# PixArt-alpha/PixArt-sigma

Hardware: AMD Instinct MI355X
Metric: denoising steps/sec (fwd+bwd) PixArt-Sigma-XL/2 1024px bs16 @1/2/4/8 GPU (higher is better)
Workload: dtype fp16; 1 GPU; PixArt-Sigma-XL/2 1024px training step (fwd+bwd+clip+AdamW), batch 16/GPU, L=300 text tokens, DP=1 RCCL all-reduce; model=PixArtMS_XL_2, global_batch=16, seq_len=4096, parallelism=dp1, grad_checkpoint=False, optimizer=adamw, text_lens=all 300

## Files before the change

### pixart_sigma_amd/csrc/gemm.hip

```cpp
#include <atomic>
#include "common.h"
#include "gemm_params.h"
#include "../../include/pixart_hip.h"
#include <cstdio>
#include <cstdlib>
#include <cstring>

namespace {
using namespace pxa;

constexpr int BM = 128, BN = 128, BK = 64;
constexpr int KC_BYTES = 128 * BK * 2;
constexpr int RC_STRIDE = (128 + 32) * 2;
constexpr int RC_BYTES = BK * RC_STRIDE;


template <bool KC>
__device__ __forceinline__ void g2r(const bf16_t* __restrict__ X, int ld, int r0, int R, int k0, int kend, uint4 (&reg)[4], int tid) {
#pragma unroll
  for (int i = 0; i < 4; i++) {
    const bf16_t* src;
    bool ok;
    if (KC) {
      int c = tid & 7, row = (tid >> 3) + 32 * i;
// ... 509 lines not shown
__device__ __forceinline__ void wait_vm_upto(int n) {
  if (n >= 6) wait_vmcnt<6>();
  else if (n == 4) wait_vmcnt<4>();
  else if (n == 2) wait_vmcnt<2>();
  else wait_vmcnt<0>();
}
#define PXA_SB() __builtin_amdgcn_sched_barrier(0)
#ifndef GEMM_ABL
#define GEMM_ABL 0
#endif
#if GEMM_ABL & 4
__device__ __forceinline__ void mfma_abl16(f32x4 (&q)[4], bf16x8 b0, bf16x8 a0, bf16x8 b1, bf16x8 a1) {
  q[0] = mfma16(b0, a0, q[0]); q[1] = mfma16(b1, a1, q[1]); q[2] = mfma16(b0, a1, q[2]); q[3] = mfma16(b1, a0, q[3]);
}
#endif
#ifndef GEMM_STORE_OVERLAP
#define GEMM_STORE_OVERLAP 1
#endif
#ifndef GEMM_M16
#define GEMM_M16 3
#endif
#ifndef GEMM_NT_STORE
#define GEMM_NT_STORE 0
#endif
#ifndef GEMM_M16_PRIO
#define GEMM_M16_PRIO 1
#endif
#ifndef GEMM_STAGGER
#define GEMM_STAGGER 0
#endif
#ifndef GEMM_EPI_EARLY
#define GEMM_EPI_EARLY 1
#endif
#ifndef GEMM_PHASE16
#define GEMM_PHASE16 -1
#endif

template <bool M16>
__device__ __forceinline__ int kc_swz(int row) { return M16 ? ((row >> 3) & 1) * 3 : (row >> 2) & 3; }
template <bool KC, bool M16 = false>
__device__ __forceinline__ const bf16_t* piece_ptr_rt(const bf16_t* __restrict__ X, int ld, int r0a, int r0b, int R, int q, int rows_log2) {
  if constexpr (KC) {
    const int row = q >> 2, c = (q & 3) ^ kc_swz<M16>(row);
    const int gr = (row < 256 ? r0a : r0b - 256) + row;
    return X + (size_t)min(gr, R - 1) * ld + c * 8;
  } else {
    const int sh = rows_log2 - 3, kr = q >> sh, cl = q & ((1 << sh) - 1);
    const int c = ((((cl >> 2) ^ (kr & 3)) << 2) | ((cl & 3) ^ (M16 ? ((kr >> 3) & 1) << 1 : 0)));
    const int col = c * 8;
    int gc = (col < 256 ? r0a : r0b - 256) + col;
    gc = gc < R ? gc : 0;
    return X + (size_t)kr * ld + gc;
  }
}
template <bool KC>
__device__ __forceinline__ bf16x8 frag_rt(const char* lds, int rbase, int ks, int lane, int rows_log2) {
  if constexpr (KC) {
    return frag_p<true, 256, 32>(lds, rbase, ks, lane);
  } else {
    const int gg = lane >> 4, tt = lane & 15, hi2 = gg >> 1;
    const int kr = ks * 16 + 8 * hi2 + (tt >> 2), col = rbase + 16 * (gg & 1) + (tt & 3) * 4;
    const int blk = col >> 5, inblk = (col & 31) * 2;
    const char* p0 = lds + (kr << (rows_log2 + 1)) + ((blk ^ (kr & 3)) << 6) + inblk;
    const char* p1 = lds + ((kr + 4) << (rows_log2 + 1)) + ((blk ^ ((kr + 4) & 3)) << 6) + inblk;
    return concat_tr(lds_tr_read(p0), lds_tr_read(p1));
  }
// ... 5 lines not shown
}
template <bool KC>
__device__ __forceinline__ bf16x8 frag16(const char* lds, int rbase, int lane, int rows_log2) {
  if constexpr (KC) {
    return frag16_kc(lds, rbase, lane);
  } else {
    const int gg = lane >> 4, tt = lane & 15;
    const int kr = 8 * gg + (tt >> 2), col = rbase + (tt & 3) * 4;
    const int blk = col >> 5, inblk = ((col & 31) * 2) ^ ((gg & 1) << 5);
    const char* p0 = lds + (kr << (rows_log2 + 1)) + ((blk ^ (kr & 3)) << 6) + inblk;
    const char* p1 = lds + ((kr + 4) << (rows_log2 + 1)) + ((blk ^ ((kr + 4) & 3)) << 6) + inblk;
    return concat_tr(lds_tr_read(p0), lds_tr_read(p1));
  }
}

#ifndef GEMM_TRACE
#define GEMM_TRACE 0
#endif
#if GEMM_TRACE
__device__ unsigned long long g_trace[12][8];
#define PXA_TR(k) do { if (blockIdx.x == 8 && tid == 0 && tr_i < 12) g_trace[tr_i][k] = __builtin_readcyclecounter(); } while (0)
#else
#define PXA_TR(k) do {} while (0)
#endif
__device__ unsigned g_sched[64][16];
__device__ unsigned g_sched_word[64][512];

template <int LAYOUT, int EPI, int RM, bool SEG = false>
__global__ __launch_bounds__(512) void gemm_pers_kernel(GemmParams p) {
  constexpr bool A_KC = (LAYOUT != 2), B_KC = (LAYOUT == 0);
  constexpr int NW = 8, TM = 4, TN = 2, BKT = 32, H1 = 2;
  constexpr bool PH16 = GEMM_PHASE16 < 0 ? (LAYOUT != 0) : (GEMM_PHASE16 != 0);
  constexpr bool M16 = ((GEMM_M16 >> LAYOUT) & 1) && !(GEMM_ABL & 4);
  constexpr int UNIT = 40960;
  extern __shared__ __attribute__((aligned(16))) char smem[];
  const int tid = threadIdx.x, lane = tid & 63, wave = __builtin_amdgcn_readfirstlane(tid >> 6), wm = wave >> 2, wn = wave & 3, hi = lane >> 5;
  const bool late = wave >= NW / 2;
  char* stg = smem + 3 * UNIT + wave * 4096;
  const int mt = (p.M + 255) / 256, ntf = p.N / 256, remn = p.N - ntf * 256;
  constexpr bool PAIR = (RM == 1), HALF = (RM == 2);
  const bool remcol = RM != 0 && remn > 0 && remn <= 128;
  const int ntp = remcol ? ntf : (p.N + 255) / 256;
  const int rem_pg = remcol ? (PAIR ? 4 : 8) : 0;
  const int per_group = 8 * ntp + rem_pg, tiles = mt * ntp + (remcol ? (PAIR ? (mt + 1) / 2 : mt) : 0), T = tiles * p.split;
  auto units_of = [&](int z) { return (min(p.K, (z + 1) * p.k_per_split) - z * p.k_per_split) / BKT; };

  int m0a = 0, m0b = 0, n0 = 0, z_ = 0;
  bool vt = false;
  const int xq = T / 8, xr = T % 8;
  auto xs = [&](int x) { return x * xq + min(x, xr); };
  auto xc = [&](int x) { return xq + (x < xr ? 1 : 0); };
  auto locate_g = [&](int Lg) {
    z_ = Lg / tiles;
    const int t = Lg - z_ * tiles;
    const int g = t / per_group, in_g = t - g * per_group, first_m = g * 8, gsz = min(mt - first_m, 8), nfull = gsz * ntp;
    if (in_g < nfull) { vt = false; m0a = (first_m + in_g % gsz) * 256; m0b = m0a; n0 = (in_g / gsz) * 256; }
    else if (PAIR) { vt = true; m0a = (first_m + 2 * (in_g - nfull)) * 256; m0b = m0a + 256; n0 = ntf * 256; }
    else if (HALF) { vt = true; m0a = (first_m + (in_g - nfull)) * 256; m0b = m0a; n0 = ntf * 256; }
  };
  const bool rev = LAYOUT != 2 && p.desc != 0;
  auto pos_of = [&](int x, int i) { return xs(x) + (rev ? xc(x) - 1 - i : i); };
  auto locate = [&](int L) { locate_g(pos_of(L % 8, L / 8)); };
  const bool DYN = p.sched_slot >= 0;
  const int myx = blockIdx.x % 8;
  unsigned* sched = g_sched[p.sched_slot & 63];
  unsigned* sched_lds = reinterpret_cast<unsigned*>(smem + 32768);
  unsigned* sched_glb = &g_sched_word[p.sched_slot & 63][blockIdx.x & 511];
  auto publish = [&](int v) {
    if (PAIR) { if (lane == 0) __hip_atomic_store(sched_glb, (unsigned)v, __ATOMIC_RELAXED, __HIP_MEMORY_SCOPE_AGENT); wait_vmcnt<0>(); }
    else { if (lane == 0) sched_lds[0] = (unsigned)v; asm volatile("s_waitcnt lgkmcnt(0)" ::: "memory"); }
  };
// ... 84 lines not shown
  auto issue_lo = [&]() __attribute__((always_inline)) {
#pragma unroll
    for (int i = 0; i < H1; i++) piece(i, s_lo);
    if (SEG) PXA_SEG_ADVANCE(seg_left0, tap_kx0, tap_ky0, tap_half0, pp[0], pp[1]);
    s_lo = (s_lo + 1) & 3;
  };
  auto issue_hi = [&]() __attribute__((always_inline)) {
    piece(2, s_hi);
    if (!(HALF && vt_pf)) piece(3, s_hi);
    if (PAIR && vt_pf) piece(4, s_hi);
    if (SEG && PAIR) { if (vt_pf) PXA_SEG_ADVANCE(seg_left1, tap_kx1, tap_ky1, tap_half1, pp[2], pp[3]); }
    s_hi = (s_hi + 1) & 3;
  };
#undef PXA_SEG_ADVANCE
  auto prefetch = [&]() __attribute__((always_inline)) {
    vt_pf = (RM != 0) && vt;
    const long k0 = (long)z_ * p.k_per_split;
    const bool vq = PAIR && vt, hq = HALF && vt;
    const int rla = vq ? 9 : 8, rlb = (vq || hq) ? 7 : 8;
    const int ln = opaque<LAYOUT == 1 || (EPI >= 2 && EPI != 7) || (GEMM_EPI_EARLY && RM == 2)>(lane);
#pragma unroll
    for (int i = 0; i < 5; i++) {
      const int id = wave + NW * i;
      const bool is_a = vq ? (i < 4) : (i < 2);
      const int pid = is_a ? id : (vq ? id - 32 : id - 16);
      if (vq || (hq ? i < 3 : i < 4)) {
        if (is_a) pp[i] = piece_ptr_rt<A_KC, M16>(p.A, p.lda, m0a, m0b, p.M, pid * 64 + ln, rla) + (A_KC ? k0 : k0 * p.lda);
        else pp[i] = piece_ptr_rt<B_KC, M16>(p.B, p.ldb, n0, n0, p.N, pid * 64 + ln, rlb) + (B_KC ? k0 : k0 * p.ldb);
      }
      st[i] = is_a ? stepA : stepB;
      dof[i] = (is_a ? 0 : (vq ? 32768 : 16384)) + pid * 1024;
    }
    s_lo = s_hi = 0;
    dma_count = 0;
    if (SEG) { seg_left0 = seg_left1 = p.k_seg; tap_kx0 = tap_kx1 = tap_ky0 = tap_ky1 = tap_half0 = tap_half1 = 0; }
    issue_lo(); issue_hi(); issue_lo(); issue_hi();
    if (nk_pf > 2) { issue_lo(); if (PH16) issue_hi(); }
  };
  prefetch();
  int tr_i = 0; (void)tr_i;
  int prev_stores = 0;

  while (true) {
    f32x16 acc[TM][TN];
    f32x4 acc4[2 * TM][2 * TN];
#pragma unroll
    for (int i = 0; i < TM; i++)
#pragma unroll
      for (int j = 0; j < TN; j++)
#pragma unroll
        for (int g = 0; g < 16; g++) acc[i][j][g] = 0.f;
#pragma unroll
    for (int i = 0; i < 2 * TM; i++)
#pragma unroll
      for (int j = 0; j < 2 * TN; j++) acc4[i][j] = f32x4{0.f, 0.f, 0.f, 0.f};
#if GEMM_ABL & 4
    f32x4 a4[TM][TN][4];
#pragma unroll
    for (int i = 0; i < TM; i++)
#pragma unroll
      for (int j = 0; j < TN; j++)
#pragma unroll
        for (int q = 0; q < 4; q++) a4[i][j][q] = f32x4{0.f, 0.f, 0.f, 0.f};
#endif
    const bool vtc = PAIR && vt, hfc = HALF && vt;
    const int a_rb = hfc ? (wave >> 1) * 64 : (vtc ? (wn >> 1) * 256 : 0) + wm * 128, b_rb = (vtc || hfc) ? (wn & 1) * 64 : wn * 64;
    const int rla = vtc ? 9 : 8, rlb = (vtc || hfc) ? 7 : 8, boff = vtc ? 32768 : 16384;
    const int mw = hfc ? m0a + a_rb : ((vtc && (wn >> 1)) ? m0b : m0a) + wm * 128, nw = n0 + b_rb;
    const int tm_eff = hfc ? 2 : TM;
    const int zw = z_;
    PXA_TR(0);
    if (GEMM_STORE_OVERLAP && LAYOUT != 2 && EPI != 3) {
      if (prev_stores == 40) wait_vmcnt<40>();
      else if (prev_stores == 36) wait_vmcnt<36>();
      else if (prev_stores == 32) wait_vmcnt<32>();
      else if (prev_stores == 28) wait_vmcnt<28>();
      else if (prev_stores == 24) wait_vmcnt<24>();
      else if (prev_stores == 20) wait_vmcnt<20>();
      else if (prev_stores == 16) wait_vmcnt<16>();
      else if (prev_stores == 12) wait_vmcnt<12>();
      else if (prev_stores == 8) wait_vmcnt<8>();
      else wait_vmcnt<0>();
    } else {
      wait_vmcnt<0>();
    }
    if (DYN && wave == 0) {
      publish(fetch_resolve());
    }
    __builtin_amdgcn_s_barrier();
    if (DYN) nxt = receive();
    if (late) __builtin_amdgcn_s_barrier();
    PXA_TR(1);
    constexpr bool EARLY = GEMM_EPI_EARLY && M16 && LAYOUT != 2;
    constexpr bool AUXA = EARLY && (EPI == 2 || EPI == 4 || EPI == 6) && !(GEMM_ABL & 16);
    typedef unsigned u32x2 __attribute__((ext_vector_type(2)));
    u32x2 axa[2][2][4];
    f32x4 bq[2 * TN];
    const bool has_bias = EARLY && p.bias != nullptr;
    auto bias_issue = [&]() {
      const int R4b = lane >> 4;
#pragma unroll
      for (int jn = 0; jn < 2 * TN; jn++) {
        const float* src = p.bias + min(nw + jn * 16 + 4 * R4b, p.N - 4);
        asm volatile("global_load_dwordx4 %0, %1, off" : "=v"(bq[jn]) : "v"(src) : "memory");
      }
    };
    auto aux_issue = [&](int i, u32x2 (&dst)[2][4]) {
      const int R4a = lane >> 4, c16a = lane & 15;
#pragma unroll
      for (int mh = 0; mh < 2; mh++)
#pragma unroll
        for (int jn = 0; jn < 4; jn++) {
          const int m = min(mw + i * 32 + 16 * mh + c16a, p.M - 1), n = min(nw + jn * 16 + 4 * R4a, p.N - 4);
          const bf16_t* src = p.aux + (size_t)m * p.ldaux + n;
          asm volatile("global_load_dwordx2 %0, %1, off" : "=v"(dst[mh][jn]) : "v"(src) : "memory");
        }
    };
    auto unit16 = [&](int t, auto rem_c, auto th_c) {
      constexpr int REM = decltype(rem_c)::value, TH = decltype(th_c)::value;
      const char* sA = smem + (t & 3) * UNIT;
      const char* sB = sA + boff;
      if constexpr (M16) {
        bf16x8 bq[2 * TN], aq[4 * TH];
#pragma unroll
        for (int j = 0; j < 2 * TN; j++) bq[j] = frag16<B_KC>(sB, b_rb + j * 16, lane, rlb);
#pragma unroll
        for (int i = 0; i < 4 * TH; i++) aq[i] = frag16<A_KC>(sA, a_rb + i * 16, lane, rla);
        if (REM >= 3) { issue_lo(); issue_hi(); }
        if (REM >= 3) { if (vtc) wait_vmcnt<10>(); else if (TH == 1) wait_vmcnt<6>(); else wait_vmcnt<8>(); }
        else if (REM == 2) { if (vtc) wait_vmcnt<5>(); else if (TH == 1) wait_vmcnt<3>(); else wait_vmcnt<4>(); }
        else if (REM == 1) wait_vmcnt<0>();
        asm volatile("s_waitcnt lgkmcnt(0)" ::: "memory");
        PXA_SB(); __builtin_amdgcn_s_barrier(); PXA_SB();
        if (GEMM_M16_PRIO && LAYOUT != 1) __builtin_amdgcn_s_setprio(1);
#pragma unroll
        for (int i = 0; i < 4 * TH; i++)
#pragma unroll
          for (int j = 0; j < 2 * TN; j++) acc4[i][j] = mfma16(bq[j], aq[i], acc4[i][j]);
        if (GEMM_M16_PRIO && LAYOUT != 1) __builtin_amdgcn_s_setprio(0);
        PXA_SB(); __builtin_amdgcn_s_barrier(); PXA_SB();
        return;
      }
      bf16x8 af[2][2 * TH], bf[2][TN];
#pragma unroll
      for (int ks = 0; ks < 2; ks++)
#pragma unroll
        for (int j = 0; j < TN; j++) bf[ks][j] = frag_rt<B_KC>(sB, b_rb + j * 32, ks, lane, rlb);
#pragma unroll
      for (int ks = 0; ks < 2; ks++)
#pragma unroll
        for (int i = 0; i < 2 * TH; i++) af[ks][i] = frag_rt<A_KC>(sA, a_rb + i * 32, ks, lane, rla);
      if (REM >= 3) { issue_lo(); issue_hi(); }
      if (REM >= 3) { if (vtc) wait_vmcnt<10>(); else if (TH == 1) wait_vmcnt<6>(); else wait_vmcnt<8>(); }
      else if (REM == 2) { if (vtc) wait_vmcnt<5>(); else if (TH == 1) wait_vmcnt<3>(); else wait_vmcnt<4>(); }
      else if (REM == 1) wait_vmcnt<0>();
      asm volatile("s_waitcnt lgkmcnt(0)" ::: "memory");
      PXA_SB(); __builtin_amdgcn_s_barrier(); PXA_SB();
      __builtin_amdgcn_s_setprio(1);
#if GEMM_ABL & 4
#pragma unroll
      for (int i = 0; i < 2 * TH; i++)
#pragma unroll
        for (int j = 0; j < TN; j++) mfma_abl16(a4[i][j], bf[0][j], af[0][i], bf[1][j], af[1][i]);
#else
#pragma unroll
      for (int ks = 0; ks < 2; ks++)
#pragma unroll
        for (int i = 0; i < 2 * TH; i++)
#pragma unroll
          for (int j = 0; j < TN; j++) acc[i][j] = mfma32(bf[ks][j], af[ks][i], acc[i][j]);
#endif
      __builtin_amdgcn_s_setprio(0);
      PXA_SB(); __builtin_amdgcn_s_barrier(); PXA_SB();
    };
    auto unit8 = [&](int t, auto rem_c, auto th_c) {
      constexpr int REM = decltype(rem_c)::value, TH = decltype(th_c)::value;
      const char* sA = smem + (t & 3) * UNIT;
      const char* sB = sA + boff;
      auto rest_a = [&]() { if (REM >= 2) issue_hi(); };
      auto rest_b = [&]() {
        if (REM >= 3) issue_lo();
        if (REM >= 3) { if (vtc) wait_vmcnt<7>(); else if (TH == 1) wait_vmcnt<5>(); else wait_vmcnt<6>(); }
        else if (REM == 2) { if (vtc) wait_vmcnt<5>(); else if (TH == 1) wait_vmcnt<3>(); else wait_vmcnt<4>(); }
        else if (REM == 1) wait_vmcnt<0>();
      };
      if constexpr (M16) {
        bf16x8 bq[2 * TN];
#pragma unroll
        for (int j = 0; j < 2 * TN; j++) bq[j] = frag16<B_KC>(sB, b_rb + j * 16, lane, rlb);
#pragma unroll
        for (int h = 0; h < 2; h++) {
          bf16x8 aq[2 * TH];
#pragma unroll
          for (int i = 0; i < 2 * TH; i++) aq[i] = frag16<A_KC>(sA, a_rb + (h * 2 * TH + i) * 16, lane, rla);
          if (h == 0) rest_a(); else rest_b();
          PXA_SB(); __builtin_amdgcn_s_barrier(); PXA_SB();
          if (GEMM_M16_PRIO) __builtin_amdgcn_s_setprio(1);
#pragma unroll
          for (int i = 0; i < 2 * TH; i++)
#pragma unroll
            for (int j = 0; j < 2 * TN; j++) acc4[h * 2 * TH + i][j] = mfma16(bq[j], aq[i], acc4[h * 2 * TH + i][j]);
          if (GEMM_M16_PRIO) __builtin_amdgcn_s_setprio(0);
          PXA_SB(); __builtin_amdgcn_s_barrier(); PXA_SB();
        }
        return;
      }
      bf16x8 af[2][TH], bf[2][TN];
#pragma unroll
      for (int ks = 0; ks < 2; ks++)
#pragma unroll
        for (int j = 0; j < TN; j++) bf[ks][j] = frag_rt<B_KC>(sB, b_rb + j * 32, ks, lane, rlb);
#pragma unroll
      for (int h = 0; h < 2; h++) {
#pragma unroll
        for (int ks = 0; ks < 2; ks++)
#pragma unroll
          for (int i = 0; i < TH; i++) af[ks][i] = frag_rt<A_KC>(sA, a_rb + (h * TH + i) * 32, ks, lane, rla);
        if (h == 0) rest_a(); else rest_b();
        PXA_SB(); __builtin_amdgcn_s_barrier(); PXA_SB();
        __builtin_amdgcn_s_setprio(1);
#if GEMM_ABL & 4
#pragma unroll
        for (int i = 0; i < TH; i++)
#pragma unroll
          for (int j = 0; j < TN; j++) mfma_abl16(a4[h * TH + i][j], bf[0][j], af[0][i], bf[1][j], af[1][i]);
#else
#pragma unroll
        for (int ks = 0; ks < 2; ks++)
#pragma unroll
// ... 10 lines not shown
    };
    auto run_units = [&](auto th_c) {
      int t = 0;
      for (; t < nk - 3; t++) unit(t, IntC<3>{}, th_c);
      if (nk >= 3) unit(t++, IntC<2>{}, th_c);
      unit(t++, IntC<1>{}, th_c);
      unit(t++, IntC<0>{}, th_c);
    };
    if (HALF && hfc) run_units(IntC<1>{}); else run_units(IntC<2>{});
#if GEMM_ABL & 4
#pragma unroll
    for (int i = 0; i < TM; i++)
#pragma unroll
      for (int j = 0; j < TN; j++)
#pragma unroll
        for (int g = 0; g < 16; g++) acc[i][j][g] = a4[i][j][g >> 2][g & 3];
#endif
    PXA_TR(2);
    if constexpr (LAYOUT != 2) {
      if (has_bias) bias_issue();
      if constexpr (AUXA) { aux_issue(0, axa[0]); aux_issue(1, axa[1]); }
    }
    if (!late) __builtin_amdgcn_s_barrier();
    PXA_TR(3);

    bool more = false;
    int pf_ops = 0;
    auto hand_over = [&]() {
      if (DYN) {
        more = nxt >= 0;
        if (more) {
          locate_g(nxt);
          nk_pf = units_of(z_);
          prefetch();
          fetch_issue();
        }
      } else {
        L += gridDim.x;
        more = L < T;
        if (more) {
          locate(L);
          nk_pf = units_of(z_);
          prefetch();
        }
      }
      if (more) pf_ops = dma_count;
    };
    const int le = opaque<LAYOUT == 1 || (EPI >= 2 && EPI != 7) || (GEMM_EPI_EARLY && RM == 2)>(lane);
    const int srow = le & 31;
    if constexpr (LAYOUT == 2) {
      hand_over();
      PXA_TR(4);
#pragma unroll
      for (int i = 0; i < TM; i++)
#pragma unroll
        for (int j = 0; j < TN; j++) {
          if constexpr (M16) {
#pragma unroll
            for (int mh = 0; mh < 2; mh++)
#pragma unroll
              for (int nh = 0; nh < 2; nh++) {
                const f32x4 a = acc4[2 * i + mh][2 * j + nh];
                const int row = 16 * mh + (lane & 15);
                *reinterpret_cast<float4*>(stg + row * 128 + (((4 * nh + (lane >> 4)) ^ (row & 7)) << 4)) = make_float4(a[0], a[1], a[2], a[3]);
              }
          } else {
#pragma unroll
          for (int q = 0; q < 4; q++)
            *reinterpret_cast<float4*>(stg + srow * 128 + (((q * 2 + hi) ^ (srow & 7)) << 4)) =
                make_float4(acc[i][j][q * 4], acc[i][j][q * 4 + 1], acc[i][j][q * 4 + 2], acc[i][j][q * 4 + 3]);
          }
          __builtin_amdgcn_s_waitcnt(0xc07f);
#pragma unroll
          for (int t4 = 0; t4 < 4; t4++) {
            const int row = t4 * 8 + (lane >> 3), ch = lane & 7;
// ... 54 lines not shown
      else if (allowed >= 24) wait_vmcnt<24>();
      else if (allowed >= 22) wait_vmcnt<22>();
      else if (allowed >= 20) wait_vmcnt<20>();
      else if (allowed >= 16) wait_vmcnt<16>();
      else if (allowed >= 12) wait_vmcnt<12>();
      else if (allowed >= 10) wait_vmcnt<10>();
      else if (allowed >= 9) wait_vmcnt<9>();
      else if (allowed >= 8) wait_vmcnt<8>();
      else if (allowed >= 4) wait_vmcnt<4>();
      else wait_vmcnt<0>();
    };
    auto aux_ready = [&](int allowed, u32x2 (&a)[2][4]) {
      wait_allow(allowed);
      asm volatile("" : "+v"(a[0][0]), "+v"(a[0][1]), "+v"(a[0][2]), "+v"(a[0][3]), "+v"(a[1][0]), "+v"(a[1][1]), "+v"(a[1][2]), "+v"(a[1][3]));
    };
    auto aux_apply = [&](int i, const u32x2 (&a)[2][4]) {
#pragma unroll
      for (int mh = 0; mh < 2; mh++)
#pragma unroll
        for (int jn = 0; jn < 4; jn++) {
          float a0, a1, a2f, a3;
          unpack_bf16x2(a[mh][jn][0], a0, a1); unpack_bf16x2(a[mh][jn][1], a2f, a3);
          f32x4& v = acc4[2 * i + mh][jn];
          if (act == 5) { v[0] += a0; v[1] += a1; v[2] += a2f; v[3] += a3; }
          else { v[0] *= a0; v[1] *= a1; v[2] *= a2f; v[3] *= a3; }
        }
    };
    hand_over();
    if constexpr (AUXA) {
      aux_ready(8 + pf_ops, axa[0]);
      if (has_bias) bias_apply();
      aux_apply(0, axa[0]);
      if (tm_eff > 2) aux_issue(2, axa[0]);
    } else {
      if (has_bias) { wait_allow(pf_ops); bias_apply(); }
    }
    PXA_TR(4);
    auto emit = [&](int j0, auto jw_c) {
      constexpr int JW = decltype(jw_c)::value, RB = JW * 64;
      constexpr int LPR = JW * 4, RPI = 64 / LPR, NST = 4 / (3 - JW);
      static_assert(!M16 || JW == 2, "16 x 16 accumulator tiles: the wave's 64 columns are one column group");
      const int R4 = le >> 4, c16 = le & 15;
      if (!EARLY) bias_add();
      float cs[8], sq[2] = {0.f, 0.f};
#pragma unroll
      for (int e = 0; e < 8; e++) cs[e] = 0.f;
      const int st_img = want_st ? mw / p.gn_img_rows : 0, st_base = st_img * p.gn_img_rows;
      const bool want_aux = !AUXA && (act == 2 || act == 4 || act == 5);
      const bool interior_a = mw + tm_eff * 32 <= p.M && nw + 64 <= p.N;
      uint2 ax[2][JW][4];
      auto load_aux = [&](int i, uint2 (&dst)[JW][4]) {
        if constexpr ((GEMM_ABL & 16) != 0) {
#pragma unroll
          for (int a_ = 0; a_ < JW; a_++)
#pragma unroll
            for (int b_ = 0; b_ < 4; b_++) dst[a_][b_] = make_uint2(OPERAND_ONE_X2, OPERAND_ONE_X2);
        } else if constexpr (M16) {
#pragma unroll
          for (int mh = 0; mh < 2; mh++)
#pragma unroll
            for (int jn = 0; jn < 4; jn++) {
              const int m = mw + i * 32 + 16 * mh + c16, n = nw + jn * 16 + 4 * R4;
              dst[mh][jn] = (m < p.M && n < p.N) ? *reinterpret_cast<const uint2*>(p.aux + (size_t)m * p.ldaux + n) : make_uint2(0u, 0u);
            }
        } else {
        const int m = mw + i * 32 + srow;
#pragma unroll
        for (int jj = 0; jj < JW; jj++)
#pragma unroll
          for (int q = 0; q < 4; q++) {
            const int n = nw + (j0 + jj) * 32 + 8 * q + 4 * hi;
            dst[jj][q] = (m < p.M && n < p.N) ? *reinterpret_cast<const uint2*>(p.aux + (size_t)m * p.ldaux + n) : make_uint2(0u, 0u);
          }
        }
      };
      auto finish4 = [&](int pass, float (&v)[4], auto&& put_back, const uint2& a2) {
        if (pass == 0 && act == 3) {
          float g[4];
#pragma unroll
          for (int e = 0; e < 4; e++) {
            if (GEMM_ABL & 64) { g[e] = v[e]; put_back(e, v[e]); }
            else put_back(e, gelu_tanh_both(v[e], g[e]));
            v[e] = g[e];
          }
        }
        if (pass == 1) {
          if (act == 1) {
#pragma unroll
            for (int e = 0; e < 4; e++) v[e] = gelu_tanh(v[e]);
          } else if (!AUXA && (act == 2 || act == 4 || act == 5)) {
            float a0, a1, a2f, a3;
            unpack_bf16x2(a2.x, a0, a1); unpack_bf16x2(a2.y, a2f, a3);
            if (act == 2) { a0 = gelu_tanh_grad(a0); a1 = gelu_tanh_grad(a1); a2f = gelu_tanh_grad(a2f); a3 = gelu_tanh_grad(a3); }
            if (act == 5) { v[0] += a0; v[1] += a1; v[2] += a2f; v[3] += a3; }
            else { v[0] *= a0; v[1] *= a1; v[2] *= a2f; v[3] *= a3; }
          }
        }
      };
      if (want_aux) load_aux(0, ax[0]);
#pragma unroll
      for (int i = 0; i < TM; i++) {
        if (i >= tm_eff) break;
        if (want_aux && i + 1 < tm_eff) load_aux(i + 1, ax[(i + 1) & 1]);
        if constexpr (AUXA) {
          if (i == 1) {
            aux_ready(interior_a ? (tm_eff > 2 ? 8 : 0) + pf_ops + 4 : 0, axa[1]);
            aux_apply(1, axa[1]);
            if (tm_eff > 3) aux_issue(3, axa[1]);
          } else if (i == 2) {
            aux_ready(interior_a ? 16 : 0, axa[0]);
            aux_apply(2, axa[0]);
          } else if (i == 3) {
            aux_ready(interior_a ? 8 : 0, axa[1]);
            aux_apply(3, axa[1]);
          }
        }
#pragma unroll
        for (int pass = 0; pass < 2; pass++) {
          if (pass == 0 && !dual) continue;
          if constexpr (M16) {
#pragma unroll
            for (int mh = 0; mh < 2; mh++)
#pragma unroll
              for (int jn = 0; jn < 4; jn++) {
                f32x4& a = acc4[2 * i + mh][jn];
                float v[4] = {a[0], a[1], a[2], a[3]};
                finish4(pass, v, [&](int e, float x) { a[e] = x; }, ax[i & 1][mh][jn]);
                const int row = 16 * mh + c16, ch = 2 * jn + (R4 >> 1);
                *reinterpret_cast<uint2*>(stg + row * RB + ((ch ^ (row & 7)) << 4) + (R4 & 1) * 8) = pack_bf16x4(v[0], v[1], v[2], v[3]);
              }
          } else {
#pragma unroll
          for (int jj = 0; jj < JW; jj++)
#pragma unroll
            for (int q = 0; q < 4; q++) {
              const int j = j0 + jj;
              float v[4] = {acc[i][j][q * 4], acc[i][j][q * 4 + 1], acc[i][j][q * 4 + 2], acc[i][j][q * 4 + 3]};
              finish4(pass, v, [&](int e, float x) { acc[i][j][q * 4 + e] = x; }, ax[i & 1][jj][q]);
              const int ch = jj * 4 + q;
              const int sw = JW == 2 ? (srow & 7) : ((srow >> 1) & 3);
              *reinterpret_cast<uint2*>(stg + srow * RB + ((ch ^ sw) << 4) + hi * 8) = pack_bf16x4(v[0], v[1], v[2], v[3]);
            }
          }
          __builtin_amdgcn_s_waitcnt(0xc07f);
          bf16_t* dst = pass == 0 ? p.out2 : p.out;
#pragma unroll
          for (int t4 = 0; t4 < NST; t4++) {
            const int row = t4 * RPI + le / LPR, ch = le % LPR;
            const int sw = JW == 2 ? (row & 7) : ((row >> 1) & 3);
            const uint4 v4 = *reinterpret_cast<const uint4*>(stg + row * RB + ((ch ^ sw) << 4));
            const int mm = mw + i * 32 + row, nn = nw + j0 * 32 + ch * 8;
            size_t orow = (size_t)mm;
            bool st_ok = mm < p.M && nn < p.N && !((GEMM_ABL & 32) && pass == 0);
            if constexpr (want_st) {
              if (p.up_rp) {
                const int pixu = mm - st_base, pyu = (int)(((float)pixu + 0.5f) * p.gn_inv_rp), pxu = pixu - pyu * p.gn_rp;
                st_ok = st_ok && pyu >= 1 && pyu <= p.gn_h && pxu >= 1 && pxu <= p.gn_w;
                orow = (size_t)st_img * p.up_ip + (size_t)((2 * pyu - 1) * p.up_rp + 2 * pxu - 1 + p.up_off);
              }
            }
            if (st_ok) {
              if (GEMM_NT_STORE) __builtin_nontemporal_store(nt_u4{v4.x, v4.y, v4.z, v4.w}, reinterpret_cast<nt_u4*>(dst + orow * p.ldo + nn));
              else *reinterpret_cast<uint4*>(dst + orow * p.ldo + nn) = v4;
            }
            if (pass == 1 && want_cs && mm < p.M) {
              float f[8];
              unpack_bf16x8(v4, f);
#pragma unroll
              for (int e = 0; e < 8; e++) cs[e] += f[e];
            }
            if (pass == 1 && want_st && mm < p.M) {
              const int pix = mm - st_base, py = (int)(((float)pix + 0.5f) * p.gn_inv_rp), px = pix - py * p.gn_rp;
              const unsigned msk = (py >= 1 && py <= p.gn_h && px >= 1 && px <= p.gn_w) ? 0xffffffffu : 0u;
              const unsigned w0 = v4.x & msk, w1 = v4.y & msk, w2 = v4.z & msk, w3 = v4.w & msk;
              cs[0] = dot2_acc(w1, OPERAND_ONE_X2, dot2_acc(w0, OPERAND_ONE_X2, cs[0]));
              cs[1] = dot2_acc(w3, OPERAND_ONE_X2, dot2_acc(w2, OPERAND_ONE_X2, cs[1]));
              sq[0] = dot2_acc(w1, w1, dot2_acc(w0, w0, sq[0]));
              sq[1] = dot2_acc(w3, w3, dot2_acc(w2, w2, sq[1]));
            }
          }
          __builtin_amdgcn_s_waitcnt(0xc07f);
        }
      }
      static_assert(!(PAIR && (EPI == 2 || EPI == 3)), "column sums in a paired instance: guard their atomics with mw < p.M as the statistics are");
      if (want_cs) {
#pragma unroll
        for (int e = 0; e < 8; e++) {
          float v = cs[e];
          if (LPR <= 4) v += __shfl_xor(v, 4);
          v += __shfl_xor(v, 8); v += __shfl_xor(v, 16); v += __shfl_xor(v, 32);
          const int n = nw + j0 * 32 + (lane % LPR) * 8 + e;
          if (lane < LPR && n < p.N) atomicAdd(p.colsum + (size_t)((mw >> 7) % PXA_COLSUM_SLOTS) * p.colsum_stride + n, v);
        }
      }
      if (want_st && mw < p.M) {
        float* dst = p.gn_part + ((size_t)((mw >> 7) % PXA_COLSUM_SLOTS) * p.gn_B + st_img) * (p.N / 4) * 2;
#pragma unroll
        for (int h = 0; h < 2; h++) {
          float v = cs[h], u = sq[h];
          if (LPR <= 4) { v += __shfl_xor(v, 4); u += __shfl_xor(u, 4); }
          v += __shfl_xor(v, 8); v += __shfl_xor(v, 16); v += __shfl_xor(v, 32);
          u += __shfl_xor(u, 8); u += __shfl_xor(u, 16); u += __shfl_xor(u, 32);
          const int n = nw + j0 * 32 + (lane % LPR) * 8 + 4 * h;
          if (lane < LPR && n < p.N) { atomicAdd(dst + (n >> 2) * 2, v); atomicAdd(dst + (n >> 2) * 2 + 1, u); }
        }
      }
    };
    if (GEMM_ABL & 2) {
      float sacc = 0.f;
#pragma unroll
      for (int i = 0; i < TM; i++)
#pragma unroll
        for (int j = 0; j < TN; j++) sacc += acc[i][j][0] + acc[i][j][7] + acc[i][j][15];
      if (sacc == 123.456f) p.out[lane] = (bf16_t)sacc;
    } else {
#pragma unroll
      for (int j0 = 0; j0 + 1 < TN; j0 += 2) emit(j0, IntC<2>{});
      if constexpr (TN % 2 == 1) emit(TN - 1, IntC<1>{});
    }
    PXA_TR(5);
#if GEMM_TRACE
    tr_i++;
#endif
    {
      const bool interior = mw + tm_eff * 32 <= p.M && nw + 64 <= p.N;
      prev_stores = (interior && p.out && !(want_st && p.up_rp)) ? tm_eff * 4 * ((dual && !(GEMM_ABL & 32)) ? 2 : 1) + (want_st ? 4 : 0) + (want_cs ? 8 : 0) + ((AUXA && tm_eff > 2) ? 16 : 0) : 0;
    }
    nk = nk_pf;
    if (!more) break;
  }
  if (DYN && wave == 0 && lane == 0 && atomicAdd(&sched[8], 1u) == gridDim.x - 1)
    for (int k = 0; k < 9; k++) sched[k] = 0u;
}

struct GemmKnobs { bool no_staged, no_pers, no_half, seg_half; int tile; bool ascending, no_glds; };
GemmKnobs read_gemm_knobs() {
  static const bool no_staged = getenv("PXA_GEMM_NO_STAGED_EPILOGUE") != nullptr;
  static const bool no_pers = getenv("PXA_GEMM_NO_PERSISTENT") != nullptr;
  static const bool no_half = getenv("PXA_GEMM_NO_HALF_ITEMS") != nullptr;
  static const bool seg_half = getenv("PXA_GEMM_SEG_HALF") != nullptr;
  static const int tile = [] { const char* f = getenv("PXA_GEMM_TILE"); return f ? atoi(f) * (strstr(f, "x128") ? -1 : 1) : 0; }();
  static const bool ascending = getenv("PXA_GEMM_ASCENDING") != nullptr;
  return GemmKnobs{no_staged, no_pers, no_half, seg_half, tile, ascending, getenv("PXA_GEMM_NO_GLDS") != nullptr};
}
int dynamic_items_env() { return getenv("PXA_GEMM_STATIC") ? 0 : getenv("PXA_GEMM_DYNAMIC") ? 1 : -1; }
std::atomic<int> g_dynamic_items{-1}; std::atomic<unsigned> g_launch_seq{0};
bool dynamic_items() {
  int expect = -1;
  if (g_dynamic_items.load(std::memory_order_relaxed) < 0) g_dynamic_items.compare_exchange_strong(expect, dynamic_items_env() == 1 ? 1 : 0);
  return g_dynamic_items.load(std::memory_order_relaxed) != 0;
}
bool pers_halfcol(int N) { return N % 256 > 0 && N % 256 <= 128; }
int pers_tiles(int M, int N, int rm) {
  const int mt = (M + 255) / 256, ntf = N / 256;
  if (rm == 2 && pers_halfcol(N)) return mt * ntf + mt;
  const bool pairing = rm == 1 && pers_halfcol(N);
  return mt * (pairing ? ntf : (N + 255) / 256) + (pairing ? (mt + 1) / 2 : 0);
}
void cost_model(int M, int N, int K, int& split, int& tile) {
  struct Cfg { int tile, bm, bn, slots; double rate; };
  const Cfg cfgs[2] = {{128, 128, 128, 512, 760e12}, {256, 256, 256, 256, 1050e12}};
// ... 64 lines not shown
}
enum class GemmFamily { simple, glds, pers };
enum GldsEpi { GLDS_DIRECT = 0, GLDS_STAGED = 1 };
enum PersEpi { PERS_PLAIN = 0, PERS_GELU_SAVE_GRAD = 1, PERS_MUL_AUX_COLSUM = 2, PERS_GENERIC = 3, PERS_ADD_AUX = 4, PERS_STATS = 5, PERS_ADD_AUX_STATS = 6, PERS_GELU = 7 };
struct GemmPlan {
  GemmFamily family; int layout, tile, epi, rm;
  bool seg; int split;
  bool try_nt4;
  bool colsum_pass_after;
};
int choose_gemm(const GemmParams& p, int layout, int split, int tile_hint, const GemmKnobs& k, GemmPlan& g) {
  g = GemmPlan{GemmFamily::simple, layout, 0, 0, 0, p.k_seg != 0, p.k_seg ? 1 : split, false, false};
  const bool bf16_only = p.out && !p.outf, hc = pers_halfcol(p.N);
  if (p.k_seg) {
    if (layout != 0) return -2;
    if (bf16_only && (p.act == 0 || p.act == 5) && p.M >= 1024 && p.N >= 128 && p.N % 128 == 0 && p.k_seg % 32 == 0 && !k.no_pers) {
      const bool pair = hc && !k.seg_half && p.M >= 512;
      g.family = GemmFamily::pers; g.rm = pair ? 1 : hc ? 2 : 0;
      g.epi = p.gn_part ? (p.act == 5 ? PERS_ADD_AUX_STATS : PERS_STATS) : (p.act == 5 ? PERS_ADD_AUX : PERS_PLAIN);
      return 0;
    }
    if (p.gn_part) { pxa_set_error("pxa_gemm: gn_part needs the persistent implicit-convolution path (bf16 output, M >= 1024, N a multiple of 128)"); return -1; }
    g.family = GemmFamily::glds; g.epi = bf16_only && p.act == 0 ? GLDS_STAGED : GLDS_DIRECT;
    return 0;
  }
  if (p.K % BK != 0 || p.k_per_split % BK != 0 || k.no_glds) { g.colsum_pass_after = p.colsum != nullptr; return 0; }
  const int want = k.tile ? k.tile : tile_hint ? tile_hint : (p.M >= 1024 && p.N >= 1024) ? 256 : 128, tile = want == 128 ? 0 : want == -256 ? 1 : 2;
  const bool pers_ok = tile == 2 && !k.no_pers;
  if (layout != 2 && pers_ok && split == 1 && bf16_only) {
    const bool half = hc && !k.no_half;
    g.family = GemmFamily::pers; g.try_nt4 = layout == 0 && p.act == 0 && !p.colsum;
    if (p.act == 0 && !p.colsum) { g.epi = PERS_PLAIN; g.rm = half ? 2 : 0; }
    else if (p.act == 3 && !p.colsum) g.epi = PERS_GELU_SAVE_GRAD;
    else if (p.act == 4 && p.colsum) { g.epi = PERS_MUL_AUX_COLSUM; g.rm = half ? 2 : 0; }
    else if (layout == 0 && p.act == 1 && !p.out2 && !p.colsum && !half) g.epi = PERS_GELU;
    else g.epi = PERS_GENERIC;
    return 0;
  }
  if (layout == 2 && pers_ok && p.outf && !p.out && !p.bias && p.act == 0 && p.accumulate != 1 && !p.colsum) { g.family = GemmFamily::pers; g.rm = hc ? 1 : 0; return 0; }
  const bool dual = (p.act == 1 && p.out2 != nullptr) || p.act == 3;
  g.family = GemmFamily::glds; g.tile = tile;
  g.epi = layout != 2 && bf16_only && !dual && !k.no_staged ? GLDS_STAGED : GLDS_DIRECT;
  g.colsum_pass_after = g.epi == GLDS_DIRECT && p.colsum != nullptr;
  return 0;
}
int plan_gemm(const pxa_gemm_args* a, GemmParams& p, GemmPlan& g) {
  const GemmKnobs k = read_gemm_knobs();
  int tile;
  const int rc = fill_gemm(a, k, p, tile);
  return rc ? rc : choose_gemm(p, a->layout, p.split, tile, k, g);
}

template <int LAYOUT, int EPI, int RM, bool SEG>
int launch_pers(GemmParams p, int split, hipStream_t s) {
  static_assert(!SEG || LAYOUT == 0, "segmented A: layout NT");
  p.split = split; constexpr int LDSP = 4 * 40960;
  hipError_t e = lds_optin(reinterpret_cast<const void*>(gemm_pers_kernel<LAYOUT, EPI, RM, SEG>), LDSP);
  if (e != hipSuccess) { pxa_set_error("hipFuncSetAttribute(gemm_pers<%d,%d>): %s", LAYOUT, EPI, hipGetErrorString(e)); return -3; }
  static int n_cu = 0;
  if (!n_cu) {
    int dev = 0; hipDeviceProp_t prop;
    if (hipGetDevice(&dev) != hipSuccess || hipGetDeviceProperties(&prop, dev) != hipSuccess) { pxa_set_error("gemm_pers: device query failed"); return -3; }
    n_cu = prop.multiProcessorCount;
  }
  const int tiles = pers_tiles(p.M, p.N, RM) * split;
  p.sched_slot = dynamic_items() ? (int)(g_launch_seq.fetch_add(1u) & 63u) : -1;
  hipLaunchKernelGGL((gemm_pers_kernel<LAYOUT, EPI, RM, SEG>), dim3(tiles < n_cu ? tiles : n_cu), dim3(512), LDSP, s, p);
// ... 99 lines not shown
```

Measured before the change: 2.400 steps/s.

## Prefetch epilogue aux operand into a rotating LDS ring via DMA

For the persistent GEMM multiply-by-aux-with-colsum epilogue, the aux tile is now loaded with LDS DMA during the last K-units, into freed pipeline stage slots and the staging buffer. The K-loop slot index is rotated by a per-tile ring base so the epilogue can reuse the slot freed last. This replaces the register-based early aux loads and is meant to hide aux-load latency behind the final MMA steps and cut register pressure. It adds vmcnt bookkeeping and extra LDS traffic, and falls back to the generic epilogue when aux is misaligned.

```diff
diff --git a/pixart_sigma_amd/csrc/gemm.hip b/pixart_sigma_amd/csrc/gemm.hip
--- a/pixart_sigma_amd/csrc/gemm.hip
+++ b/pixart_sigma_amd/csrc/gemm.hip
@@ -565,6 +565,9 @@
 #ifndef GEMM_EPI_EARLY
 #define GEMM_EPI_EARLY 1
 #endif
+#ifndef GEMM_AUX_RING
+#define GEMM_AUX_RING 1
+#endif
 #ifndef GEMM_PHASE16
 #define GEMM_PHASE16 -1
 #endif
@@ -636,11 +639,14 @@
   constexpr int NW = 8, TM = 4, TN = 2, BKT = 32, H1 = 2;
   constexpr bool PH16 = GEMM_PHASE16 < 0 ? (LAYOUT != 0) : (GEMM_PHASE16 != 0);
   constexpr bool M16 = ((GEMM_M16 >> LAYOUT) & 1) && !(GEMM_ABL & 4);
+  constexpr bool RING = GEMM_AUX_RING && GEMM_EPI_EARLY && M16 && LAYOUT != 2 && EPI == 2 && RM != 1 && !SEG && !(GEMM_ABL & 16);
   constexpr int UNIT = 40960;
   extern __shared__ __attribute__((aligned(16))) char smem[];
   const int tid = threadIdx.x, lane = tid & 63, wave = __builtin_amdgcn_readfirstlane(tid >> 6), wm = wave >> 2, wn = wave & 3, hi = lane >> 5;
   const bool late = wave >= NW / 2;
   char* stg = smem + 3 * UNIT + wave * 4096;
+  char* stgT = smem + (wave >> 1) * UNIT + 32768 + (wave & 1) * 4096;
+  int rb = 0, rb_pf = 0;
   const int mt = (p.M + 255) / 256, ntf = p.N / 256, remn = p.N - ntf * 256;
   constexpr bool PAIR = (RM == 1), HALF = (RM == 2);
   const bool remcol = RM != 0 && remn > 0 && remn <= 128;
@@ -791,6 +797,7 @@
       dof[i] = (is_a ? 0 : (vq ? 32768 : 16384)) + pid * 1024;
     }
     s_lo = s_hi = 0;
+    if constexpr (RING) s_lo = s_hi = rb_pf;
     dma_count = 0;
     if (SEG) { seg_left0 = seg_left1 = p.k_seg; tap_kx0 = tap_kx1 = tap_ky0 = tap_ky1 = tap_half0 = tap_half1 = 0; }
     issue_lo(); issue_hi(); issue_lo(); issue_hi();
@@ -828,6 +835,24 @@
     const int mw = hfc ? m0a + a_rb : ((vtc && (wn >> 1)) ? m0b : m0a) + wm * 128, nw = n0 + b_rb;
     const int tm_eff = hfc ? 2 : TM;
     const int zw = z_;
+    char* stgS = nullptr;
+    if constexpr (RING) stgS = smem + ((nk + rb) & 3) * UNIT + wave * 4096;
+    auto aux_dma = [&](int i, char* buf) __attribute__((always_inline)) {
+      const int r8 = lane >> 3, n = min(nw + (((lane & 7) ^ r8) << 3), p.N - 8);
+      const int off = __builtin_amdgcn_readfirstlane((int)(buf - smem));
+#pragma unroll
+      for (int q = 0; q < 4; q++) {
+        const int m = min(mw + i * 32 + q * 8 + r8, p.M - 1);
+        lds_dma16(p.aux + (size_t)m * p.ldaux + n, smem + off + q * 1024);
+      }
+    };
+    auto ring_issue = [&](auto rem_c) __attribute__((always_inline)) {
+      constexpr int REM = decltype(rem_c)::value;
+      if (REM == 2 || (REM == 1 && nk < 3)) { aux_dma(0, stgT); aux_dma(1, stgS); }
+    };
+    auto ring_wait1 = [&]() {
+      if (nk >= 3) wait_vmcnt<8>(); else wait_vmcnt<0>();
+    };
     PXA_TR(0);
     if (GEMM_STORE_OVERLAP && LAYOUT != 2 && EPI != 3) {
       if (prev_stores == 40) wait_vmcnt<40>();
@@ -851,7 +876,7 @@
     if (late) __builtin_amdgcn_s_barrier();
     PXA_TR(1);
     constexpr bool EARLY = GEMM_EPI_EARLY && M16 && LAYOUT != 2;
-    constexpr bool AUXA = EARLY && (EPI == 2 || EPI == 4 || EPI == 6) && !(GEMM_ABL & 16);
+    constexpr bool AUXA = EARLY && (EPI == 2 || EPI == 4 || EPI == 6) && !(GEMM_ABL & 16) && !RING;
     typedef unsigned u32x2 __attribute__((ext_vector_type(2)));
     u32x2 axa[2][2][4];
     f32x4 bq[2 * TN];
@@ -877,7 +902,9 @@
     };
     auto unit16 = [&](int t, auto rem_c, auto th_c) {
       constexpr int REM = decltype(rem_c)::value, TH = decltype(th_c)::value;
-      const char* sA = smem + (t & 3) * UNIT;
+      int slot = t & 3;
+      if constexpr (RING) slot = (t + rb) & 3;
+      const char* sA = smem + slot * UNIT;
       const char* sB = sA + boff;
       if constexpr (M16) {
         bf16x8 bq[2 * TN], aq[4 * TH];
@@ -888,9 +915,10 @@
         if (REM >= 3) { issue_lo(); issue_hi(); }
         if (REM >= 3) { if (vtc) wait_vmcnt<10>(); else if (TH == 1) wait_vmcnt<6>(); else wait_vmcnt<8>(); }
         else if (REM == 2) { if (vtc) wait_vmcnt<5>(); else if (TH == 1) wait_vmcnt<3>(); else wait_vmcnt<4>(); }
-        else if (REM == 1) wait_vmcnt<0>();
+        else if (REM == 1) { if constexpr (RING) ring_wait1(); else wait_vmcnt<0>(); }
         asm volatile("s_waitcnt lgkmcnt(0)" ::: "memory");
         PXA_SB(); __builtin_amdgcn_s_barrier(); PXA_SB();
+        if constexpr (RING) ring_issue(rem_c);
         if (GEMM_M16_PRIO && LAYOUT != 1) __builtin_amdgcn_s_setprio(1);
 #pragma unroll
         for (int i = 0; i < 4 * TH; i++)
@@ -934,14 +962,16 @@
     };
     auto unit8 = [&](int t, auto rem_c, auto th_c) {
       constexpr int REM = decltype(rem_c)::value, TH = decltype(th_c)::value;
-      const char* sA = smem + (t & 3) * UNIT;
+      int slot = t & 3;
+      if constexpr (RING) slot = (t + rb) & 3;
+      const char* sA = smem + slot * UNIT;
       const char* sB = sA + boff;
       auto rest_a = [&]() { if (REM >= 2) issue_hi(); };
       auto rest_b = [&]() {
         if (REM >= 3) issue_lo();
         if (REM >= 3) { if (vtc) wait_vmcnt<7>(); else if (TH == 1) wait_vmcnt<5>(); else wait_vmcnt<6>(); }
         else if (REM == 2) { if (vtc) wait_vmcnt<5>(); else if (TH == 1) wait_vmcnt<3>(); else wait_vmcnt<4>(); }
-        else if (REM == 1) wait_vmcnt<0>();
+        else if (REM == 1) { if constexpr (RING) ring_wait1(); else wait_vmcnt<0>(); }
       };
       if constexpr (M16) {
         bf16x8 bq[2 * TN];
@@ -954,6 +984,7 @@
           for (int i = 0; i < 2 * TH; i++) aq[i] = frag16<A_KC>(sA, a_rb + (h * 2 * TH + i) * 16, lane, rla);
           if (h == 0) rest_a(); else rest_b();
           PXA_SB(); __builtin_amdgcn_s_barrier(); PXA_SB();
+          if constexpr (RING) { if (h == 1) ring_issue(rem_c); }
           if (GEMM_M16_PRIO) __builtin_amdgcn_s_setprio(1);
 #pragma unroll
           for (int i = 0; i < 2 * TH; i++)
@@ -1030,6 +1061,7 @@
         if (more) {
           locate_g(nxt);
           nk_pf = units_of(z_);
+          if constexpr (RING) rb_pf = __builtin_amdgcn_readfirstlane((nk + rb + 1) & 3);
           prefetch();
           fetch_issue();
         }
@@ -1039,6 +1071,7 @@
         if (more) {
           locate(L);
           nk_pf = units_of(z_);
+          if constexpr (RING) rb_pf = __builtin_amdgcn_readfirstlane((nk + rb + 1) & 3);
           prefetch();
         }
       }
@@ -1159,6 +1192,9 @@
       if (has_bias) bias_apply();
       aux_apply(0, axa[0]);
       if (tm_eff > 2) aux_issue(2, axa[0]);
+    } else if constexpr (RING) {
+      wait_allow(has_bias ? pf_ops : 4 + pf_ops);
+      if (has_bias) bias_apply();
     } else {
       if (has_bias) { wait_allow(pf_ops); bias_apply(); }
     }
@@ -1173,7 +1209,7 @@
 #pragma unroll
       for (int e = 0; e < 8; e++) cs[e] = 0.f;
       const int st_img = want_st ? mw / p.gn_img_rows : 0, st_base = st_img * p.gn_img_rows;
-      const bool want_aux = !AUXA && (act == 2 || act == 4 || act == 5);
+      const bool want_aux = !AUXA && !RING && (act == 2 || act == 4 || act == 5);
       const bool interior_a = mw + tm_eff * 32 <= p.M && nw + 64 <= p.N;
       uint2 ax[2][JW][4];
       auto load_aux = [&](int i, uint2 (&dst)[JW][4]) {
@@ -1215,7 +1251,7 @@
           if (act == 1) {
 #pragma unroll
             for (int e = 0; e < 4; e++) v[e] = gelu_tanh(v[e]);
-          } else if (!AUXA && (act == 2 || act == 4 || act == 5)) {
+          } else if (!AUXA && !RING && (act == 2 || act == 4 || act == 5)) {
             float a0, a1, a2f, a3;
             unpack_bf16x2(a2.x, a0, a1); unpack_bf16x2(a2.y, a2f, a3);
             if (act == 2) { a0 = gelu_tanh_grad(a0); a1 = gelu_tanh_grad(a1); a2f = gelu_tanh_grad(a2f); a3 = gelu_tanh_grad(a3); }
@@ -1242,6 +1278,24 @@
             aux_apply(3, axa[1]);
           }
         }
+        char* stg_i = stg;
+        if constexpr (RING) {
+          stg_i = (i & 1) ? stgS : stgT;
+          if (i == 1) wait_allow(pf_ops + (interior_a ? 4 : 0) + (tm_eff > 2 ? 4 : 0));
+          else if (i == 2) wait_allow((interior_a ? 4 : 0) + (tm_eff > 3 ? 4 : 0));
+          else if (i == 3) wait_allow(interior_a ? 4 : 0);
+#pragma unroll
+          for (int mh = 0; mh < 2; mh++)
+#pragma unroll
+            for (int jn = 0; jn < 4; jn++) {
+              const int row = 16 * mh + c16, ch = 2 * jn + (R4 >> 1);
+              const uint2 a2 = *reinterpret_cast<const uint2*>(stg_i + row * RB + ((ch ^ (row & 7)) << 4) + (R4 & 1) * 8);
+              float a0, a1, a2f, a3;
+              unpack_bf16x2(a2.x, a0, a1); unpack_bf16x2(a2.y, a2f, a3);
+              f32x4& v = acc4[2 * i + mh][jn];
+              v[0] *= a0; v[1] *= a1; v[2] *= a2f; v[3] *= a3;
+            }
+        }
 #pragma unroll
         for (int pass = 0; pass < 2; pass++) {
           if (pass == 0 && !dual) continue;
@@ -1254,7 +1308,7 @@
                 float v[4] = {a[0], a[1], a[2], a[3]};
                 finish4(pass, v, [&](int e, float x) { a[e] = x; }, ax[i & 1][mh][jn]);
                 const int row = 16 * mh + c16, ch = 2 * jn + (R4 >> 1);
-                *reinterpret_cast<uint2*>(stg + row * RB + ((ch ^ (row & 7)) << 4) + (R4 & 1) * 8) = pack_bf16x4(v[0], v[1], v[2], v[3]);
+                *reinterpret_cast<uint2*>(stg_i + row * RB + ((ch ^ (row & 7)) << 4) + (R4 & 1) * 8) = pack_bf16x4(v[0], v[1], v[2], v[3]);
               }
           } else {
 #pragma unroll
@@ -1266,7 +1320,7 @@
               finish4(pass, v, [&](int e, float x) { acc[i][j][q * 4 + e] = x; }, ax[i & 1][jj][q]);
               const int ch = jj * 4 + q;
               const int sw = JW == 2 ? (srow & 7) : ((srow >> 1) & 3);
-              *reinterpret_cast<uint2*>(stg + srow * RB + ((ch ^ sw) << 4) + hi * 8) = pack_bf16x4(v[0], v[1], v[2], v[3]);
+              *reinterpret_cast<uint2*>(stg_i + srow * RB + ((ch ^ sw) << 4) + hi * 8) = pack_bf16x4(v[0], v[1], v[2], v[3]);
             }
           }
           __builtin_amdgcn_s_waitcnt(0xc07f);
@@ -1275,7 +1329,7 @@
           for (int t4 = 0; t4 < NST; t4++) {
             const int row = t4 * RPI + le / LPR, ch = le % LPR;
             const int sw = JW == 2 ? (row & 7) : ((row >> 1) & 3);
-            const uint4 v4 = *reinterpret_cast<const uint4*>(stg + row * RB + ((ch ^ sw) << 4));
+            const uint4 v4 = *reinterpret_cast<const uint4*>(stg_i + row * RB + ((ch ^ sw) << 4));
             const int mm = mw + i * 32 + row, nn = nw + j0 * 32 + ch * 8;
             size_t orow = (size_t)mm;
             bool st_ok = mm < p.M && nn < p.N && !((GEMM_ABL & 32) && pass == 0);
@@ -1308,6 +1362,7 @@
           }
           __builtin_amdgcn_s_waitcnt(0xc07f);
         }
+        if constexpr (RING) { if (i + 2 < tm_eff) aux_dma(i + 2, stg_i); }
       }
       static_assert(!(PAIR && (EPI == 2 || EPI == 3)), "column sums in a paired instance: guard their atomics with mw < p.M as the statistics are");
       if (want_cs) {
@@ -1351,9 +1406,10 @@
 #endif
     {
       const bool interior = mw + tm_eff * 32 <= p.M && nw + 64 <= p.N;
-      prev_stores = (interior && p.out && !(want_st && p.up_rp)) ? tm_eff * 4 * ((dual && !(GEMM_ABL & 32)) ? 2 : 1) + (want_st ? 4 : 0) + (want_cs ? 8 : 0) + ((AUXA && tm_eff > 2) ? 16 : 0) : 0;
+      prev_stores = (interior && p.out && !(want_st && p.up_rp)) ? tm_eff * 4 * ((dual && !(GEMM_ABL & 32)) ? 2 : 1) + (want_st ? 4 : 0) + (want_cs ? 8 : 0) + ((AUXA && tm_eff > 2) ? 16 : 0) + ((RING && tm_eff > 2) ? 8 : 0) : 0;
     }
     nk = nk_pf;
+    if constexpr (RING) rb = rb_pf;
     if (!more) break;
   }
   if (DYN && wave == 0 && lane == 0 && atomicAdd(&sched[8], 1u) == gridDim.x - 1)
@@ -1484,7 +1540,7 @@
     g.family = GemmFamily::pers; g.try_nt4 = layout == 0 && p.act == 0 && !p.colsum;
     if (p.act == 0 && !p.colsum) { g.epi = PERS_PLAIN; g.rm = half ? 2 : 0; }
     else if (p.act == 3 && !p.colsum) g.epi = PERS_GELU_SAVE_GRAD;
-    else if (p.act == 4 && p.colsum) { g.epi = PERS_MUL_AUX_COLSUM; g.rm = half ? 2 : 0; }
+    else if (p.act == 4 && p.colsum && !(GEMM_AUX_RING && (p.ldaux % 8 != 0 || (reinterpret_cast<uintptr_t>(p.aux) & 15) != 0))) { g.epi = PERS_MUL_AUX_COLSUM; g.rm = half ? 2 : 0; }
     else if (layout == 0 && p.act == 1 && !p.out2 && !p.colsum && !half) g.epi = PERS_GELU;
     else g.epi = PERS_GENERIC;
     return 0;
```

Measured after the change: 2.406 steps/s (median of 6 runs). No clear change (+0.3%).
